# ModelTC/llmc

Measured on AMD Instinct MI355X. Metric: layers/sec (GPTQ W4A16, Llama-3-8B Linear shapes, 128x2048 calib), higher is better.
Workload: dtype bf16

## Files before the change

llmc_amd/csrc/abi.hip:

```cpp
#include <mutex>
#include <set>
#include <utility>
#include "common.h"

namespace llmc {
static thread_local char g_last_error[512] = "";
static thread_local int g_helper_streams = 1;
bool helper_streams_enabled() { return g_helper_streams != 0; }
static thread_local int g_cu_reserve = 0;
int cu_reserve() { return g_cu_reserve; }
static thread_local int g_opt[OPT_COUNT] = {};
int opt(int id) { return (id >= 0 && id < OPT_COUNT) ? g_opt[id] : 0; }
static const char* const g_opt_names[OPT_COUNT] = {
    "k3_fp32", "k3_no_gemm6", "k3_no_planes", "k3_split_far", "k4_split_far", "k4_err_rowmajor", "gptq_generic",
    "gemm3_nospec", "gemm3s_min_tiles", "no_shortk", "linear_nosplit", "fp8_exact_div", "side_cu_mask", "k1_batch_off", "k1_fp32_diag", "fp8_no_packed16", "gemm3s_no_dma", "sgemm_no_wide", "gemm3_no_wide", "no_riders"};

void set_last_error(const char* where, hipError_t e) {
    snprintf(g_last_error, sizeof(g_last_error), "%s: %s (%d)", where, hipGetErrorString(e), (int)e);
}
void set_last_error_msg(const char* msg) { snprintf(g_last_error, sizeof(g_last_error), "%s", msg); }

static std::mutex g_dev_mu;
static int g_cu_count[LLMC_MAX_DEVICES] = {};
static std::set<std::pair<int, const void*>> g_lds_attr_done;

int device_cu_count() {
    int dev = 0;
    if (hipGetDevice(&dev) != hipSuccess || dev < 0 || dev >= LLMC_MAX_DEVICES) return 256;
    std::lock_guard<std::mutex> lk(g_dev_mu);
    if (g_cu_count[dev] == 0) {
        int n = 0;
        if (hipDeviceGetAttribute(&n, hipDeviceAttributeMultiprocessorCount, dev) != hipSuccess || n <= 0) n = 256;
        g_cu_count[dev] = n;
    }
    return g_cu_count[dev];
}

int ensure_dynamic_lds(const void* fn, int bytes) {
    int dev = 0;
    LLMC_HIP_CHECK(hipGetDevice(&dev));
    std::lock_guard<std::mutex> lk(g_dev_mu);
    auto key = std::make_pair(dev, fn);
    if (g_lds_attr_done.count(key)) return LLMC_OK;
    LLMC_HIP_CHECK(hipFuncSetAttribute(fn, hipFuncAttributeMaxDynamicSharedMemorySize, bytes));
    g_lds_attr_done.insert(key);
    return LLMC_OK;
}
}

extern "C" int llmc_hip_set_helper_streams(int enable) {
    int prev = llmc::g_helper_streams;
    llmc::g_helper_streams = enable ? 1 : 0;
    return prev;
}

extern "C" int llmc_hip_set_option(const char* key, int value) {
    if (!key || value < 0) return LLMC_EINVAL;
    for (int i = 0; i < llmc::OPT_COUNT; ++i)
        if (strcmp(key, llmc::g_opt_names[i]) == 0) {
            const int prev = llmc::g_opt[i];
            llmc::g_opt[i] = value;
            return prev;
        }
    llmc::set_last_error_msg("llmc_hip_set_option: unknown key");
    return LLMC_EINVAL;
}

extern "C" int llmc_hip_get_option(const char* key) {
    if (!key) return LLMC_EINVAL;
    for (int i = 0; i < llmc::OPT_COUNT; ++i)
        if (strcmp(key, llmc::g_opt_names[i]) == 0) return llmc::g_opt[i];
    return LLMC_EINVAL;
}

extern "C" int llmc_hip_option_name(int index, char* buf_host, size_t n) {
    if (index < 0 || index >= llmc::OPT_COUNT || !buf_host || n == 0) return LLMC_EINVAL;
    strncpy(buf_host, llmc::g_opt_names[index], n - 1);
    buf_host[n - 1] = 0;
    return (int)strlen(buf_host);
}

extern "C" int llmc_hip_set_cu_reserve(int n_cus) {
    int prev = llmc::g_cu_reserve;
    llmc::g_cu_reserve = n_cus < 0 ? 0 : n_cus;
    return prev;
}

extern "C" int llmc_hip_abi_version(void) { return LLMC_HIP_ABI_VERSION; }

#ifndef LLMC_BUILD_ID
#define LLMC_BUILD_ID "unknown"
#endif
extern "C" const char* llmc_hip_build_id(void) { return LLMC_BUILD_ID; }

extern "C" int llmc_hip_last_error(char* buf_host, size_t n) {
    if (!buf_host || n == 0) return (int)strlen(llmc::g_last_error);
    strncpy(buf_host, llmc::g_last_error, n - 1);
    buf_host[n - 1] = 0;
    return (int)strlen(buf_host);
}
```

llmc_amd/csrc/common.h:

```cpp
#pragma once
#include <hip/hip_runtime.h>
#include <stdint.h>
#include <string.h>
#include <stdio.h>
#include <stdlib.h>

#include "../../include/llmc_hip.h"

namespace llmc {

void set_last_error(const char* where, hipError_t e);
void set_last_error_msg(const char* msg);

#define LLMC_HIP_CHECK(expr)                                   \
    do {                                                       \
        hipError_t _e = (expr);                                \
        if (_e != hipSuccess) {                                \
            ::llmc::set_last_error(#expr, _e);                 \
            return LLMC_EIO;                                   \
        }                                                      \
    } while (0)

#define LLMC_LAUNCH_CHECK()                                    \
    do {                                                       \
        hipError_t _e = hipGetLastError();                     \
        if (_e != hipSuccess) {                                \
            ::llmc::set_last_error("kernel launch", _e);       \
            return LLMC_EIO;                                   \
        }                                                      \
    } while (0)

#define LLMC_REQUIRE(cond, msg)                                \
    do {                                                       \
        if (!(cond)) {                                         \
            ::llmc::set_last_error_msg(msg);                   \
            return LLMC_EINVAL;                                \
        }                                                      \
    } while (0)

static constexpr int LLMC_MAX_DEVICES = 64;
int device_cu_count();
int ensure_dynamic_lds(const void* fn, int bytes);
int cu_reserve();
bool helper_streams_enabled();

enum Opt : int {
    OPT_K3_FP32 = 0,
    OPT_K3_NO_GEMM6,
    OPT_K3_NO_PLANES,
    OPT_K3_SPLIT_FAR,
    OPT_K4_SPLIT_FAR,
    OPT_K4_ERR_ROWMAJOR,
    OPT_GPTQ_GENERIC,
    OPT_GEMM3_NOSPEC,
    OPT_GEMM3S_MIN_TILES,
    OPT_NO_SHORTK,
    OPT_LINEAR_NOSPLIT,
    OPT_FP8_EXACT_DIV,
    OPT_SIDE_CU_MASK,
    OPT_K1_BATCH_OFF,
    OPT_K1_FP32_DIAG,
    OPT_FP8_NO_PACKED16,
    OPT_GEMM3S_NO_DMA,
    OPT_SGEMM_NO_WIDE,
    OPT_GEMM3_NO_WIDE,
    OPT_NO_RIDERS,
    OPT_COUNT
};
int opt(int id);
#ifdef LLMC_LAB
static inline const char* lab_env(const char* k) { return getenv(k); }
#endif

static inline int dtype_size(int dt) { return dt == LLMC_F32 ? 4 : 2; }
static inline bool dtype_ok(int dt) { return dt == LLMC_F16 || dt == LLMC_BF16 || dt == LLMC_F32; }

struct f16_t { uint16_t u; };
struct bf16_t { uint16_t u; };

template <typename T> struct dt_of;
template <> struct dt_of<f16_t> { static constexpr int value = LLMC_F16; };
template <> struct dt_of<bf16_t> { static constexpr int value = LLMC_BF16; };
template <> struct dt_of<float> { static constexpr int value = LLMC_F32; };

#define DISPATCH_DT(dt, ...)                                              \
    switch (dt) {                                                         \
        case LLMC_F16: { using T = ::llmc::f16_t; __VA_ARGS__; break; }   \
        case LLMC_BF16: { using T = ::llmc::bf16_t; __VA_ARGS__; break; } \
        default: { using T = float; __VA_ARGS__; break; }                 \
    }
#define DISPATCH_OUT_KIND(kind, ...)                                                     \
    switch (kind) {                                                                      \
        case LLMC_OUT_FAKE: { constexpr int KIND = LLMC_OUT_FAKE; __VA_ARGS__; break; }  \
        case LLMC_OUT_I32: { constexpr int KIND = LLMC_OUT_I32; __VA_ARGS__; break; }    \
        case LLMC_OUT_I8: { constexpr int KIND = LLMC_OUT_I8; __VA_ARGS__; break; }      \
        case LLMC_OUT_U8: { constexpr int KIND = LLMC_OUT_U8; __VA_ARGS__; break; }      \
    }

__device__ __forceinline__ float f16_bits_to_f32(uint16_t u) {
    _Float16 h;
    __builtin_memcpy(&h, &u, 2);
    return (float)h;
}
__device__ __forceinline__ uint16_t f32_to_f16_bits(float v) {
    asm volatile("" : "+v"(v));
    _Float16 h = (_Float16)v;
    uint16_t u;
    __builtin_memcpy(&u, &h, 2);
    return u;
}
__device__ __forceinline__ float bf16_bits_to_f32(uint16_t u) {
    return __uint_as_float(((uint32_t)u) << 16);
}
__device__ __forceinline__ uint16_t f32_to_bf16_bits(float v) {
    const __bf16 h = (__bf16)v;
    uint16_t u;
    __builtin_memcpy(&u, &h, 2);
    return u;
}

__device__ __forceinline__ float opaque_f32(float v) {
    asm volatile("" : "+v"(v));
    return v;
}

__device__ __forceinline__ float rnd(float v, int dt) {
    if (dt == LLMC_F16) return f16_bits_to_f32(f32_to_f16_bits(v));
    if (dt == LLMC_BF16) return bf16_bits_to_f32(f32_to_bf16_bits(v));
    return v;
}
template <int DT> __device__ __forceinline__ float rndc(float v) {
    if constexpr (DT == LLMC_F16) return f16_bits_to_f32(f32_to_f16_bits(v));
    else if constexpr (DT == LLMC_BF16) return bf16_bits_to_f32(f32_to_bf16_bits(v));
    else return v;
}

__device__ __forceinline__ float load_as_f32(const void* p, int64_t i, int dt) {
    if (dt == LLMC_F16) return f16_bits_to_f32(((const uint16_t*)p)[i]);
    if (dt == LLMC_BF16) return bf16_bits_to_f32(((const uint16_t*)p)[i]);
    return ((const float*)p)[i];
}
__device__ __forceinline__ void store_from_f32(void* p, int64_t i, int dt, float v) {
    if (dt == LLMC_F16) ((uint16_t*)p)[i] = f32_to_f16_bits(v);
    else if (dt == LLMC_BF16) ((uint16_t*)p)[i] = f32_to_bf16_bits(v);
    else ((float*)p)[i] = v;
}

template <typename T> __device__ __forceinline__ float to_f32(T v);
template <> __device__ __forceinline__ float to_f32<f16_t>(f16_t v) { return f16_bits_to_f32(v.u); }
template <> __device__ __forceinline__ float to_f32<bf16_t>(bf16_t v) { return bf16_bits_to_f32(v.u); }
template <> __device__ __forceinline__ float to_f32<float>(float v) { return v; }

template <typename T> __device__ __forceinline__ T from_f32(float v);
template <> __device__ __forceinline__ f16_t from_f32<f16_t>(float v) { return f16_t{f32_to_f16_bits(v)}; }
template <> __device__ __forceinline__ bf16_t from_f32<bf16_t>(float v) { return bf16_t{f32_to_bf16_bits(v)}; }
template <> __device__ __forceinline__ float from_f32<float>(float v) { return v; }

__host__ __device__ __forceinline__ int promote(int a, int b) {
    if (a == b) return a;
    return LLMC_F32;
}

__device__ __forceinline__ float wave_max(float v, int width) {
    for (int o = width >> 1; o > 0; o >>= 1) v = fmaxf(v, __shfl_xor(v, o, 64));
    return v;
}
__device__ __forceinline__ float wave_min(float v, int width) {
    for (int o = width >> 1; o > 0; o >>= 1) v = fminf(v, __shfl_xor(v, o, 64));
    return v;
}
__device__ __forceinline__ float wave_sum(float v, int width) {
    for (int o = width >> 1; o > 0; o >>= 1) v += __shfl_xor(v, o, 64);
    return v;
}

static inline int64_t ceil_div64(int64_t a, int64_t b) { return (a + b - 1) / b; }
static inline int capped_grid(int64_t items, int64_t per_block, int64_t cap) {
    const int64_t b = ceil_div64(items, per_block);
    return (int)(b < 1 ? 1 : (b > cap ? cap : b));
}
static inline int pow2_ceil(int64_t x) {
    int p = 1;
    while (p < x) p <<= 1;
    return p;
}

}
```

llmc_amd/csrc/gptq_loop.hip:

```cpp
#include "gptq_block_kernels.h"
#include "pipe_lanes.h"

using namespace llmc;

static constexpr int GRP = 4;
static constexpr int GW = BS * GRP;

extern "C" size_t llmc_gptq_quantize_ws_bytes(int64_t R, int64_t K) {
    if (R <= 0 || K <= 0) return 0;
    return 3 * (size_t)((R + 3) & ~(int64_t)3) * GW * sizeof(float);
}

extern "C" int llmc_gptq_quantize(float* W, const float* Hinv, int64_t R, int64_t K, int sym, float qmin,
                                  float qmax, int64_t group_size, int static_groups, const int32_t* col_group,
                                  float* scales, float* zeros, float* Wout, float* losses, int blocksize,
                                  void* ws, llmc_stream_t stream) {
    return llmc_gptq_quantize_cols(W, Hinv, R, K, K, sym, qmin, qmax, group_size, static_groups, col_group, scales,
                                   zeros, Wout, losses, blocksize, ws, stream);
}

struct MseSearch { int round_zp, nsteps, grid; float norm; };

struct Piece { int64_t c0, c1; int k0, k1; Lane lane; };
static constexpr int CARRIERS = GRP;
static_assert(CARRIERS % RIDER_PASSES == 0 && GRP % RIDER_PASSES == 0, "a group's carrying launches and phases divide into the passes");

static int far_pieces(int64_t gend, int64_t K, bool merged, int rider_cols, Piece* p) {
    const int64_t gend2 = gend + GW < K ? gend + GW : K, gend3 = gend2 + GW < K ? gend2 + GW : K;
    if (!merged) {
        p[0] = Piece{gend, gend2, 0, GW, CHAIN}, p[1] = Piece{gend2, gend3, 0, GW, BULK}, p[2] = Piece{gend3, K, 0, GW, BULK};
        return 1 + (gend2 < K) + (gend3 < K);
    }
    const int64_t rw = (int64_t)rider_cols * 128, rspan = (CARRIERS / RIDER_PASSES) * rw;
    const int64_t p0 = (rider_cols > 0 && gend2 < K) ? (gend2 > K - rspan ? gend2 : K - rspan) : K;
    p[0] = Piece{gend, p0, 0, GW, CHAIN};
    int n = 1;
    const int kd = GW / RIDER_PASSES;
    for (int pass = 0; pass < RIDER_PASSES; ++pass)
        for (int64_t c = p0; c < K; c += rw) p[n++] = Piece{c, c + rw < K ? c + rw : K, pass * kd, (pass + 1) * kd, RIDE};
    return n;
}

struct ColCall {
    float* W; const float* U; float* Wout; float* losses; float* scales; float* zeros; const int32_t* col_group;
    int64_t R, K, NQ;
    bool ekm; int64_t Rp, err_ld; float* ErrBuf[3];
    int ng, gsz, static_mode, sym; float qmin, qmax;
    const MseSearch* mse;
    int kind;

    float* err(int group, int64_t k) const { return ErrBuf[group % 3] + (ekm ? k * Rp : k); }
    int64_t group_end(int64_t g0) const { return g0 + GW < NQ ? g0 + GW : NQ; }
    int64_t near_end(int64_t g0) const { return group_end(g0) == NQ ? K : group_end(g0); }
    int count(int64_t i1) const { return (int)(NQ - i1 < BS ? NQ - i1 : BS); }

    GptqBlockArgs block(int64_t i1) const {
        GptqBlockArgs a;
        a.W = W; a.U = U; a.Wout = Wout; a.losses = losses;
        a.Err = err((int)(i1 / GW), i1 % GW); a.err_ld = (int)err_ld; a.err_kmajor = ekm ? 1 : 0;
        a.scales = scales; a.zeros = zeros; a.col_group = mse ? nullptr : col_group; a.col_gsz = mse ? gsz : 1 << 30;
        a.R = R; a.K = (int)K; a.i1 = (int)i1; a.count = count(i1); a.ng = ng; a.gsz = static_mode ? BS : gsz;
        a.static_mode = static_mode; a.sym = sym; a.qmin = qmin; a.qmax = qmax;
        return a;
    }
    SgemmArgs product(const float* A, int64_t row0, int kd, int64_t c0, int64_t c1, int phase_len) const {
        SgemmArgs g{};
        g.A = A; g.lda = err_ld; g.B = U + row0 * K + c0; g.ldb = K; g.C = W + c0; g.ldc = K;
        g.M = g.M_last = (int)R; g.N = g.N_last = (int)(c1 - c0); g.Kd = g.Kd_last = kd;
        g.epilogue = SG_SUB; g.batch = 1; g.phase_len = phase_len;
        return g;
    }
    SgemmArgs near(int64_t i1) const {
        const int64_t g0 = i1 - i1 % GW, c0 = (i1 + count(i1)) & ~(int64_t)3;
        return product(err((int)(i1 / GW), i1 % GW), i1, count(i1), c0, near_end(g0), 0);
    }
    SgemmArgs far(int group, int64_t c0, int64_t c1, int k0, int k1) const {
        return product(err(group, k0), (int64_t)group * GW + k0, k1 - k0, c0, c1, BS);
    }
    RiderArgs riders(int group, const Piece& q, int nchain) const {
        RiderArgs ra{};
        wide::wide_operands<2>(far(group, q.c0, q.c1, q.k0, q.k1), ra.w);
        ra.nchain = nchain; ra.per = (nchain % 8 == 0 && ra.w.tm % 8 == 0) ? ra.w.tm / 8 : 0;
        return ra;
    }
};

enum { PLAN_BLOCK = 0, PLAN_NEAR = 1, PLAN_NEAR_FAR = 2, PLAN_FAR = 3, PLAN_FLUSH = 4, PLAN_W = 12 };
static const int32_t PLAN_BLANK[PLAN_W] = {0, 0, 0, 0, -1, -1, -1, 0, 0, -1, 0, 0};

struct Sink {
    const ColCall& o; const Lanes& ln; PlanRec* rec;
    void add(int lane, int kind, int group, int64_t w0, int64_t w1, int err_rd, int err_wr, int rgroup, int64_t r0, int64_t r1, int rerr,
             int k0, int k1) const {
        const int32_t v[PLAN_W] = {kind, group, (int32_t)w0, (int32_t)w1, err_rd, err_wr, rgroup, (int32_t)r0, (int32_t)r1, rerr, k0, k1};
        rec->row(v, lane);
    }
    int err_index(const float* pe) const { return (int)((size_t)(pe - o.ErrBuf[0]) / ((size_t)o.Rp * GW)); }
    void k_range(int group, const float* B, int64_t c0, int kd, int* k0, int* k1) const {
        *k0 = (int)((B - o.U - c0) / o.K - (int64_t)group * GW);
        *k1 = *k0 + kd;
        if (kd == GW) *k0 = *k1 = 0;
    }
    int product(int kind, int group, const SgemmArgs& g, hipStream_t st) const {
        if (!rec) return sgemm_launch(g, o.ekm, false, st);
        const int64_t c0 = g.C - o.W;
        int k0 = 0, k1 = 0;
        if (kind != PLAN_NEAR) k_range(group, g.B, c0, g.Kd, &k0, &k1);
        add(ln.lane_of(st), kind, group, c0, c0 + g.N, err_index(g.A), -1, -1, 0, 0, -1, k0, k1);
        return LLMC_OK;
    }
    int in_block(int group, const GptqBlockArgs& a, int variant, int nt, int grid, const RiderArgs* ra, int rgroup) const {
        const hipStream_t st = ln.s[CHAIN];
        if (rec) {
            int64_t r0 = 0, r1 = 0;
            int rerr = -1, k0 = 0, k1 = 0;
            if (ra) {
                r0 = ra->w.C - o.W, r1 = r0 + (int64_t)ra->w.tn * 128, rerr = err_index(ra->w.A);
                k_range(rgroup, ra->w.B, r0, ra->w.nst * wide::W_K, &k0, &k1);
            }
            add(CHAIN, PLAN_BLOCK, group, a.i1, a.i1 + a.count, -1, err_index(a.Err), rgroup, r0, r1, rerr, k0, k1);
            return LLMC_OK;
        }
        return o.kind == QK_E4M3 ? gptq_launch_in_block_e4m3(a, variant, nt, grid, ra, st)
             : o.kind == QK_E5M2 ? gptq_launch_in_block_e5m2(a, variant, nt, grid, ra, st)
                                 : launch_in_block<QK_INT>(a, variant, nt, grid, ra, st);
    }
};

static int rider_quota(const ColCall& o, bool merged, int nt, int grid) {
    if (!merged || opt(OPT_NO_RIDERS) || !o.ekm || nt != GBT || o.R % 128 || o.K % 128 || o.NQ <= GW || o.K <= 2 * (int64_t)GW) return 0;
    const int free_cus = device_cu_count() - grid;
    if (sgemm_route(o.far(0, 2 * GW, o.K, 0, GW), true, false).wide_form != 2 || free_cus <= 0 || 2 * grid < device_cu_count()) return 0;
    return (int)(free_cus / (o.R / 128));
}

static int gptq_cols_impl(float* W, const float* Hinv, int64_t R, int64_t K, int64_t n_quant, int sym, float qmin,
                          float qmax, int64_t group_size, int static_groups, const int32_t* col_group, float* scales,
                          float* zeros, float* Wout, float* losses, int blocksize, void* ws, llmc_stream_t stream,
                          const MseSearch* mse, PlanRec* rec = nullptr, int kind = QK_INT) {
    LLMC_REQUIRE(W && Hinv && Wout && scales && ws && R > 0 && K > 0, "gptq_quantize: null/empty argument");
    LLMC_REQUIRE(n_quant > 0 && n_quant <= K, "gptq_quantize: n_quant must be in (0, K]");
    LLMC_REQUIRE(blocksize == BS, "gptq_quantize: blocksize must be 128");
    LLMC_REQUIRE(K % 4 == 0 && K < (1 << 30), "gptq_quantize: K must be a multiple of 4");
    LLMC_REQUIRE(sym || zeros, "gptq_quantize: zeros required for asymmetric");
    const bool per_channel = group_size <= 0;
    const int static_mode = static_groups || per_channel || mse != nullptr;
    const int gsz = (int)group_size;
    if (!static_mode || mse) {
        if (!(gsz == 16 || gsz == 32 || gsz == 64 || gsz == 128)) {
            set_last_error_msg("gptq_quantize: dynamic group qparams need group_size in {16,32,64,128}");
            return LLMC_ENOTSUP;
        }
    } else if (!per_channel) {
        LLMC_REQUIRE(col_group != nullptr, "gptq_quantize: col_group required with static groups");
    }
    const bool ekm = !opt(OPT_K4_ERR_ROWMAJOR);
    const int64_t Rp = (R + 3) & ~(int64_t)3;
    const ColCall o{W, Hinv, Wout, losses, scales, zeros, per_channel ? nullptr : col_group, R, K, n_quant,
                    ekm, Rp, ekm ? Rp : GW, {(float*)ws, (float*)ws + (size_t)Rp * GW, (float*)ws + 2 * (size_t)Rp * GW},
                    per_channel ? 1 : (int)ceil_div64(K, group_size), gsz, static_mode, sym, qmin, qmax, mse, kind};
    Lanes ln((hipStream_t)stream, rec);
    const Sink sink{o, ln, rec};
    const bool merged = !ln.piped() && !opt(OPT_K4_SPLIT_FAR);
    const int nt = R >= 16384 ? 1024 : GBT;
    const int grid = (int)ceil_div64(R, nt / 16);
    const int rider_cols = rider_quota(o, merged, nt, grid);
    const bool force_generic = opt(OPT_GPTQ_GENERIC) != 0;
    Piece pc[1 + CARRIERS];
    int np = 0, next = 0, fg = 0;
    auto flush = [&]() -> int {
        for (; next < np; ++next)
            LLMC_TRY(sink.product(PLAN_FLUSH, fg, o.far(fg, pc[next].c0, pc[next].c1, pc[next].k0, pc[next].k1), ln.s[CHAIN]));
        return LLMC_OK;
    };
    Ev reached_next{};
    Ev err_read[3] = {};
    Ev bulk_tail{};
    LLMC_TRY(ln.fork());
    int g = 0;
    for (int64_t g0 = 0; g0 < o.NQ; g0 += GW, ++g) {
        const int64_t gend = o.group_end(g0), near_end = o.near_end(g0);
        if (near_end > gend) {
            LLMC_TRY(flush());
            LLMC_TRY(ln.wait(CHAIN, bulk_tail));
        }
        LLMC_TRY(ln.wait(CHAIN, err_read[g % 3]));
        for (int64_t i1 = g0; i1 < gend; i1 += BS) {
            const GptqBlockArgs a = o.block(i1);
            const int variant = (a.count != BS || force_generic) ? 0 : static_mode ? 1 : gsz == BS ? BS : 0;
            if (mse && !rec) {
                LLMC_TRY(llmc_mse_qparams_panel(W, R, K, i1, a.count, gsz, sym, mse->round_zp, qmin, qmax, mse->nsteps, mse->grid,
                                                mse->norm, scales, zeros, o.ng, i1 / gsz, (llmc_stream_t)ln.s[CHAIN]));
            }
            const bool ride = next < np;
            const RiderArgs ra = ride ? o.riders(fg, pc[next++], grid) : RiderArgs{};
            LLMC_TRY(sink.in_block(g, a, variant, nt, grid, ride ? &ra : nullptr, ride ? fg : -1));
            if (i1 + a.count < near_end) LLMC_TRY(sink.product(PLAN_NEAR, g, o.near(i1), ln.s[CHAIN]));
        }
        if (near_end == K) continue;
        LLMC_TRY(ln.wait(CHAIN, reached_next));
        reached_next = Ev{};
        LLMC_TRY(flush());
        np = far_pieces(gend, K, merged, rider_cols, pc);
        fg = g;
        int nbulk = 0;
        for (next = 0; next < np && pc[next].lane != RIDE; ++next) {
            const Piece& p = pc[next];
            if (p.lane == BULK && nbulk == 0) LLMC_TRY(ln.order(CHAIN, BULK));
            const int kind = (p.lane == CHAIN && !merged) ? PLAN_NEAR_FAR : PLAN_FAR;
            LLMC_TRY(sink.product(kind, g, o.far(g, p.c0, p.c1, p.k0, p.k1), ln.s[p.lane]));
            if (p.lane == BULK && nbulk++ == 0) LLMC_TRY(ln.record(BULK, &reached_next));
        }
        if (nbulk) {
            LLMC_TRY(ln.record(BULK, &err_read[g % 3]));
            bulk_tail = err_read[g % 3];
        }
    }
    LLMC_TRY(flush());
    return ln.join();
}

extern "C" int llmc_gptq_quantize_cols(float* W, const float* Hinv, int64_t R, int64_t K, int64_t n_quant, int sym,
                                       float qmin, float qmax, int64_t group_size, int static_groups,
                                       const int32_t* col_group, float* scales, float* zeros, float* Wout,
                                       float* losses, int blocksize, void* ws, llmc_stream_t stream) {
    return gptq_cols_impl(W, Hinv, R, K, n_quant, sym, qmin, qmax, group_size, static_groups, col_group, scales, zeros,
                          Wout, losses, blocksize, ws, stream, nullptr);
}

extern "C" int llmc_gptq_quantize_fp8_cols(float* W, const float* Hinv, int64_t R, int64_t K, int64_t n_quant, int fmt,
                                           int64_t group_size, int static_groups, const int32_t* col_group, float* scales,
                                           float* Wout, float* losses, int blocksize, void* ws, llmc_stream_t stream) {
    if (fmt != 0 && fmt != 1) {
        set_last_error_msg("gptq_quantize_fp8_cols: fmt must be 0 (e4m3) or 1 (e5m2)");
        return LLMC_ENOTSUP;
    }
    const float qmax = fmt ? 57344.0f : 448.0f;
    return gptq_cols_impl(W, Hinv, R, K, n_quant, 1, -qmax, qmax, group_size, static_groups, col_group, scales, nullptr, Wout,
                          losses, blocksize, ws, stream, nullptr, nullptr, fmt ? QK_E5M2 : QK_E4M3);
}

extern "C" size_t llmc_gptq_quantize_mse_ws_bytes(int64_t R, int64_t K) { return llmc_gptq_quantize_ws_bytes(R, K); }

extern "C" int llmc_gptq_quantize_mse(float* W, const float* Hinv, int64_t R, int64_t K, int64_t n_quant, int sym,
                                      float qmin, float qmax, int64_t group_size, int round_zp, int nsteps, int grid,
                                      float norm, float* scales, float* zeros, float* Wout, float* losses,
                                      int blocksize, void* ws, llmc_stream_t stream) {
    LLMC_REQUIRE(nsteps >= 1 && grid >= 1, "gptq_quantize_mse: nsteps and grid must be positive");
    if (!(group_size == 16 || group_size == 32 || group_size == 64 || group_size == 128)) {
        set_last_error_msg("gptq_quantize_mse: the searched group qparams need group_size in {16,32,64,128}");
        return LLMC_ENOTSUP;
    }
    const MseSearch m{round_zp, nsteps, grid, norm};
    return gptq_cols_impl(W, Hinv, R, K, n_quant, sym, qmin, qmax, group_size, 0, nullptr, scales, zeros, Wout, losses,
                          blocksize, ws, stream, &m);
}

static int gptq_plan(int64_t R, int64_t K, int64_t n_quant, int64_t group_size, int static_groups, int32_t* out, int cap, bool lanes) {
    LLMC_REQUIRE(out && cap >= 0, "gptq plan: null output");
    PlanRec rec{out, cap, 0, PLAN_W, lanes, PLAN_BLANK};
    float* const base = (float*)(uintptr_t)((uint64_t)1 << 40);
    const size_t span = (size_t)1 << 36;
    int32_t* cg = (int32_t*)(base + 6 * span);
    int rc = gptq_cols_impl(base, base + span, R, K, n_quant, 0, 0.0f, 15.0f, group_size, static_groups, cg, base + 2 * span,
                            base + 3 * span, base + 4 * span, nullptr, BS, base + 5 * span, nullptr, nullptr, &rec);
    return rc ? rc : rec.n;
}
extern "C" int llmc_test_gptq_rider_plan(int64_t R, int64_t K, int64_t n_quant, int64_t group_size, int static_groups, int32_t* out, int cap) {
    return gptq_plan(R, K, n_quant, group_size, static_groups, out, cap, false);
}
extern "C" int llmc_test_gptq_pipe_plan(int64_t R, int64_t K, int64_t n_quant, int64_t group_size, int static_groups, int32_t* out, int cap) {
    return gptq_plan(R, K, n_quant, group_size, static_groups, out, cap, true);
}
```

Measured before the change: 78.58.

## Add tall-matrix GPTQ block kernel with several lanes per row for large R

Adds a new in-block GPTQ kernel for tall weight matrices (R >= 16384 by default, INT quantization, whole blocks). Each row is split across 8 lanes that exchange values through DPP broadcasts, and the block's U tile is staged in padded LDS. The intent is better parallelism and register use than the existing per-row kernel on matrices with many rows. Riders are turned off when this path is taken, which gives up the overlap of far-update work inside the block kernel. A fast path with a fallback handles non-finite or non-positive values.

```diff
diff --git a/llmc_amd/csrc/abi.hip b/llmc_amd/csrc/abi.hip
--- a/llmc_amd/csrc/abi.hip
+++ b/llmc_amd/csrc/abi.hip
@@ -13,7 +13,8 @@
 int opt(int id) { return (id >= 0 && id < OPT_COUNT) ? g_opt[id] : 0; }
 static const char* const g_opt_names[OPT_COUNT] = {
     "k3_fp32", "k3_no_gemm6", "k3_no_planes", "k3_split_far", "k4_split_far", "k4_err_rowmajor", "gptq_generic",
-    "gemm3_nospec", "gemm3s_min_tiles", "no_shortk", "linear_nosplit", "fp8_exact_div", "side_cu_mask", "k1_batch_off", "k1_fp32_diag", "fp8_no_packed16", "gemm3s_no_dma", "sgemm_no_wide", "gemm3_no_wide", "no_riders"};
+    "gemm3_nospec", "gemm3s_min_tiles", "no_shortk", "linear_nosplit", "fp8_exact_div", "side_cu_mask", "k1_batch_off", "k1_fp32_diag", "fp8_no_packed16", "gemm3s_no_dma", "sgemm_no_wide", "gemm3_no_wide", "no_riders",
+    "k4_tall_off", "k4_tall_min_rows"};
 
 void set_last_error(const char* where, hipError_t e) {
     snprintf(g_last_error, sizeof(g_last_error), "%s: %s (%d)", where, hipGetErrorString(e), (int)e);
diff --git a/llmc_amd/csrc/common.h b/llmc_amd/csrc/common.h
--- a/llmc_amd/csrc/common.h
+++ b/llmc_amd/csrc/common.h
@@ -65,6 +65,8 @@
     OPT_SGEMM_NO_WIDE,
     OPT_GEMM3_NO_WIDE,
     OPT_NO_RIDERS,
+    OPT_K4_TALL_OFF,
+    OPT_K4_TALL_MIN_ROWS,
     OPT_COUNT
 };
 int opt(int id);
diff --git a/llmc_amd/csrc/gptq_block_tall.h b/llmc_amd/csrc/gptq_block_tall.h
--- /dev/null
+++ b/llmc_amd/csrc/gptq_block_tall.h
@@ -0,0 +1,224 @@
+#pragma once
+#include <utility>
+#include "gptq_block_kernels.h"
+
+namespace llmc {
+
+static constexpr int TALL_NT = 512;
+static constexpr int TALL_RS = BS + 4 * (BS / 32);
+static constexpr int TALL_LDS = BS * TALL_RS * 4 + BS * (int)sizeof(float2) + 16;
+template <int LPR> __host__ __device__ constexpr int tall_seg(int p) { return p * (BS / LPR) + 4 * ((p * (BS / LPR)) >> 5); }
+static constexpr int TALL_LPR = 8;
+
+template <int LPR, int PO> __device__ __forceinline__ float lpr_bcast(float v, bool hi) {
+    constexpr int Q = PO & 3;
+    const int b = __builtin_amdgcn_update_dpp(0, __float_as_int(v), Q | (Q << 2) | (Q << 4) | (Q << 6), 0xf, 0xf, false);
+    if constexpr (LPR == 4) {
+        return __int_as_float(b);
+    } else {
+        static_assert(LPR == 8, "4 or 8 lanes per row");
+        const int o = __builtin_amdgcn_update_dpp(0, b, PO < 4 ? 0x114 : 0x104, 0xf, 0xf, false);
+        return __int_as_float(PO < 4 ? (hi ? o : b) : (hi ? b : o));
+    }
+}
+
+template <int I, int LPR, bool STATIC, int KIND, bool FAST>
+__device__ __forceinline__ void tall_step(float (&w)[BS / LPR], float (&df)[BS / LPR], const float (&sc)[BS / LPR],
+                                          const float (&zr)[BS / LPR], const float* __restrict__ us,
+                                          const float2* __restrict__ dtab, int p, bool hi, float s_cur, float z_cur,
+                                          float y_cur, float qmin, float qmax) {
+    constexpr int NE = BS / LPR, PO = I % LPR, EO = I / LPR;
+    float u[NE];
+#pragma unroll
+    for (int e = EO & ~3; e < NE; e += 4) {
+        const float4 v = *reinterpret_cast<const float4*>(us + I * TALL_RS + e);
+        u[e] = v.x, u[e + 1] = v.y, u[e + 2] = v.z, u[e + 3] = v.w;
+    }
+    const float2 dd = dtab[I];
+    float s = s_cur, z = z_cur, y = y_cur;
+    if (STATIC) {
+        s = lpr_bcast<LPR, PO>(sc[EO], hi);
+        if (KIND == QK_INT) z = lpr_bcast<LPR, PO>(zr[EO], hi);
+        if (FAST) y = rcp_refined(s);
+    }
+    const float wi = lpr_bcast<LPR, PO>(w[EO], hi);
+    float q;
+    if constexpr (FAST) {
+        float t = div_tail(wi, s, y);
+        if constexpr (KIND == QK_INT) {
+            t = rintf(t);
+            t = t + z;
+            const float qc = fminf(fmaxf(t, qmin), qmax);
+            q = (qc - z) * s;
+        } else {
+            q = (KIND == QK_E4M3 ? qtorch_select_finite<4, 3>(t) : qtorch_select_finite<5, 2>(t)) * s;
+        }
+    } else if constexpr (KIND == QK_INT) {
+        const float qc = quant_code(wi, s, z, LLMC_F32, LLMC_F32, qmin, qmax);
+        q = dequant_code(qc, s, z, LLMC_F32);
+    } else {
+        q = float_qdq<KIND>(wi, s);
+    }
+    const float diff = wi - q;
+    float err;
+    if constexpr (FAST) err = div_tail(diff, dd.x, dd.y);
+    else err = diff / dd.x;
+    df[EO] = p == PO ? diff : df[EO];
+    asm volatile("" : "+v"(df[EO]));
+    typedef float v2f __attribute__((ext_vector_type(2)));
+    if (EO & 1) {
+        const float tt = err * u[EO];
+        w[EO] = w[EO] - tt;
+    }
+#pragma unroll
+    for (int e = (EO + 1) & ~1; e < NE; e += 2) {
+        const v2f uu = {u[e], u[e + 1]};
+        v2f ww = {w[e], w[e + 1]};
+        const v2f tt = uu * err;
+        ww = ww - tt;
+        w[e] = ww.x;
+        w[e + 1] = ww.y;
+    }
+    __builtin_amdgcn_sched_barrier(0);
+}
+
+template <int LPR, bool STATIC, int KIND, bool FAST, int... I>
+__device__ __forceinline__ void tall_steps(std::integer_sequence<int, I...>, float (&w)[BS / LPR], float (&df)[BS / LPR],
+                                           const float (&sc)[BS / LPR], const float (&zr)[BS / LPR],
+                                           const float* __restrict__ us, const float2* __restrict__ dtab, int p, bool hi,
+                                           float s_cur, float z_cur, float y_cur, float qmin, float qmax) {
+    (tall_step<I, LPR, STATIC, KIND, FAST>(w, df, sc, zr, us, dtab, p, hi, s_cur, z_cur, y_cur, qmin, qmax), ...);
+}
+
+template <int LPR, bool STATIC, int KIND, bool FAST>
+__device__ __forceinline__ bool tall_block(const GptqBlockArgs& a, const float* __restrict__ Us,
+                                           const float2* __restrict__ dtab, int p, bool hi, int64_t row, bool active) {
+    constexpr int NE = BS / LPR;
+    const int64_t rr = active ? row : a.R - 1;
+    float w[NE], df[NE], sc[NE], zr[NE];
+    bool bad = false;
+    float mn = INFINITY, mx = -INFINITY;
+#pragma unroll
+    for (int e = 0; e < NE; ++e) {
+        const int c = p + LPR * e;
+        w[e] = a.W[rr * a.K + a.i1 + c];
+        df[e] = 0.0f;
+        sc[e] = 1.0f;
+        zr[e] = 0.0f;
+        if (STATIC) {
+            const int g = a.col_group ? a.col_group[a.i1 + c] : (a.i1 + c) / a.col_gsz;
+            sc[e] = a.scales[rr * a.ng + g];
+            zr[e] = a.zeros ? a.zeros[rr * a.ng + g] : 0.0f;
+            if (FAST) bad |= !plain_pos(sc[e]);
+        } else {
+            mn = fminf(mn, w[e]);
+            mx = fmaxf(mx, w[e]);
+        }
+    }
+    float s_cur = 1.0f, z_cur = 0.0f, y_cur = 1.0f;
+    if (!STATIC) {
+        mn = wave_min(mn, LPR);
+        mx = wave_max(mx, LPR);
+        const QParams qp = qparams_from_minmax(mn, mx, LLMC_F32, a.sym, 1, a.qmin, a.qmax);
+        s_cur = qp.s;
+        z_cur = qp.z;
+        if (FAST) {
+            y_cur = rcp_refined(s_cur);
+            bad |= !plain_pos(s_cur);
+        }
+    }
+    tall_steps<LPR, STATIC, KIND, FAST>(std::make_integer_sequence<int, BS>{}, w, df, sc, zr, Us + tall_seg<LPR>(p), dtab, p, hi, s_cur,
+                                        z_cur, y_cur, a.qmin, a.qmax);
+    if (FAST) {
+#pragma unroll
+        for (int e = 0; e < NE; ++e) bad |= !plain_num(w[e]) | !plain_num(df[e]);
+        if (__any(bad)) return false;
+    }
+    if (!active) return true;
+#pragma unroll
+    for (int e = 0; e < NE; ++e) {
+        const int c = p + LPR * e;
+        const float2 dd = dtab[c];
+        a.Wout[row * a.K + a.i1 + c] = w[e];
+        if (a.losses) a.losses[row * a.K + a.i1 + c] = (df[e] * df[e]) / (2.0f * (dd.x * dd.x));
+        float err;
+        if constexpr (FAST) err = div_tail(df[e], dd.x, dd.y);
+        else err = df[e] / dd.x;
+        a.Err[a.err_kmajor ? (int64_t)c * a.err_ld + row : (int64_t)row * a.err_ld + c] = err;
+    }
+    if (!STATIC && p == 0) {
+        const int g = a.i1 / BS;
+        a.scales[row * a.ng + g] = s_cur;
+        if (a.zeros) a.zeros[row * a.ng + g] = z_cur;
+    }
+    return true;
+}
+
+template <int VARIANT, int LPR, int KIND = QK_INT>
+__global__ __launch_bounds__(TALL_NT) void k_gptq_block_tall(GptqBlockArgs a) {
+    static_assert(VARIANT == 1 || VARIANT == BS, "the generic variant stays on k_gptq_block");
+    constexpr bool STATIC = VARIANT == 1;
+    constexpr int NE = BS / LPR;
+    extern __shared__ __attribute__((aligned(16))) char smem_t[];
+    float* Us = reinterpret_cast<float*>(smem_t);
+    float2* dtab = reinterpret_cast<float2*>(Us + BS * TALL_RS);
+    int& d_not_plain = *reinterpret_cast<int*>(dtab + BS);
+    if (threadIdx.x == 0) d_not_plain = 0;
+    __syncthreads();
+    const int tid = threadIdx.x;
+    {
+        constexpr int NV = BS * BS / 4 / TALL_NT;
+        float4 v[NV];
+#pragma unroll
+        for (int j = 0; j < NV; ++j) {
+            const int idx = tid + TALL_NT * j;
+            const int i = idx >> 5, c4 = (idx & 31) * 4;
+            v[j] = *reinterpret_cast<const float4*>(a.U + (int64_t)(a.i1 + i) * a.K + a.i1 + c4);
+        }
+#pragma unroll
+        for (int j = 0; j < NV; ++j) {
+            const int idx = tid + TALL_NT * j;
+            const int i = idx >> 5, c4 = (idx & 31) * 4;
+            const float vv[4] = {v[j].x, v[j].y, v[j].z, v[j].w};
+#pragma unroll
+            for (int t = 0; t < 4; ++t) {
+                const int c = c4 + t;
+                if (c == i) {
+                    dtab[i] = make_float2(vv[t], rcp_refined(vv[t]));
+                    if (!plain_pos(vv[t])) d_not_plain = 1;
+                }
+                Us[i * TALL_RS + tall_seg<LPR>(c % LPR) + c / LPR] = c > i ? vv[t] : 0.0f;
+            }
+        }
+    }
+    __syncthreads();
+
+    const int lane = tid & 63;
+    const int p = lane % LPR;
+    const bool hi = (lane & 4) != 0;
+    const int64_t row = ((int64_t)blockIdx.x * (TALL_NT / 64) + (tid >> 6)) * (64 / LPR) + lane / LPR;
+    const bool active = row < a.R;
+    if (!d_not_plain && tall_block<LPR, STATIC, KIND, true>(a, Us, dtab, p, hi, row, active)) return;
+    tall_block<LPR, STATIC, KIND, false>(a, Us, dtab, p, hi, row, active);
+}
+
+template <int KIND>
+static int launch_in_block_tall(const GptqBlockArgs& a, int variant, hipStream_t st) {
+    if (a.count != BS || (variant != 1 && variant != BS)) {
+        set_last_error_msg("k_gptq_block_tall: whole blocks with given or group-128 qparams only");
+        return LLMC_EINVAL;
+    }
+    const int rows = (TALL_NT / 64) * (64 / TALL_LPR);
+    const dim3 grid((unsigned)ceil_div64(a.R, rows));
+#define LLMC_GBT(V, L)                                                                                         \
+    do {                                                                                                       \
+        if (int rc = ensure_dynamic_lds((const void*)k_gptq_block_tall<V, L, KIND>, TALL_LDS)) return rc;      \
+        hipLaunchKernelGGL((k_gptq_block_tall<V, L, KIND>), grid, dim3(TALL_NT), TALL_LDS, st, a);             \
+    } while (0)
+    if (variant == 1) LLMC_GBT(1, TALL_LPR); else LLMC_GBT(BS, TALL_LPR);
+#undef LLMC_GBT
+    LLMC_LAUNCH_CHECK();
+    return LLMC_OK;
+}
+
+}
diff --git a/llmc_amd/csrc/gptq_loop.hip b/llmc_amd/csrc/gptq_loop.hip
--- a/llmc_amd/csrc/gptq_loop.hip
+++ b/llmc_amd/csrc/gptq_loop.hip
@@ -1,4 +1,5 @@
 #include "gptq_block_kernels.h"
+#include "gptq_block_tall.h"
 #include "pipe_lanes.h"
 
 using namespace llmc;
@@ -109,7 +110,7 @@
         add(ln.lane_of(st), kind, group, c0, c0 + g.N, err_index(g.A), -1, -1, 0, 0, -1, k0, k1);
         return LLMC_OK;
     }
-    int in_block(int group, const GptqBlockArgs& a, int variant, int nt, int grid, const RiderArgs* ra, int rgroup) const {
+    int in_block(int group, const GptqBlockArgs& a, int variant, int nt, int grid, const RiderArgs* ra, int rgroup, bool tall) const {
         const hipStream_t st = ln.s[CHAIN];
         if (rec) {
             int64_t r0 = 0, r1 = 0;
@@ -121,6 +122,7 @@
             add(CHAIN, PLAN_BLOCK, group, a.i1, a.i1 + a.count, -1, err_index(a.Err), rgroup, r0, r1, rerr, k0, k1);
             return LLMC_OK;
         }
+        if (tall) return launch_in_block_tall<QK_INT>(a, variant, st);
         return o.kind == QK_E4M3 ? gptq_launch_in_block_e4m3(a, variant, nt, grid, ra, st)
              : o.kind == QK_E5M2 ? gptq_launch_in_block_e5m2(a, variant, nt, grid, ra, st)
                                  : launch_in_block<QK_INT>(a, variant, nt, grid, ra, st);
@@ -164,7 +166,9 @@
     const bool merged = !ln.piped() && !opt(OPT_K4_SPLIT_FAR);
     const int nt = R >= 16384 ? 1024 : GBT;
     const int grid = (int)ceil_div64(R, nt / 16);
-    const int rider_cols = rider_quota(o, merged, nt, grid);
+    const int tall_min_rows = opt(OPT_K4_TALL_MIN_ROWS) > 0 ? opt(OPT_K4_TALL_MIN_ROWS) : 16384;
+    const bool tall = kind == QK_INT && R >= tall_min_rows && !opt(OPT_K4_TALL_OFF);
+    const int rider_cols = tall ? 0 : rider_quota(o, merged, nt, grid);
     const bool force_generic = opt(OPT_GPTQ_GENERIC) != 0;
     Piece pc[1 + CARRIERS];
     int np = 0, next = 0, fg = 0;
@@ -194,7 +198,7 @@
             }
             const bool ride = next < np;
             const RiderArgs ra = ride ? o.riders(fg, pc[next++], grid) : RiderArgs{};
-            LLMC_TRY(sink.in_block(g, a, variant, nt, grid, ride ? &ra : nullptr, ride ? fg : -1));
+            LLMC_TRY(sink.in_block(g, a, variant, nt, grid, ride ? &ra : nullptr, ride ? fg : -1, tall && variant != 0));
             if (i1 + a.count < near_end) LLMC_TRY(sink.product(PLAN_NEAR, g, o.near(i1), ln.s[CHAIN]));
         }
         if (near_end == K) continue;
```

Result: no change. 79.07 (median of 6 runs) (+0.6%).
